# ittiam-systems/libxaac

Measured on AMD Instinct MI355X. Metric: decoded audio frames/s (1024-spl IMDCT + complex QMF + HQ SBR + parametric stereo, HE-AACv2), higher is better.
Workload: dtype int32

## Files before the change

### libxaac_amd/csrc/fx.h

```cpp
#ifndef XAAC_FX_H
#define XAAC_FX_H

#include <stdint.h>

#if defined(__HIPCC__)
#define FX_HD __host__ __device__ __forceinline__
#define FX_MEMBER __host__ __device__ __forceinline__
#else
#define FX_HD static inline
#define FX_MEMBER inline
#endif

#define FX_MAX32 ((int32_t)0x7fffffff)
#define FX_MIN32 ((int32_t)0x80000000)

FX_HD int32_t fx_add(int32_t a, int32_t b) { return (int32_t)((uint32_t)a + (uint32_t)b); }
FX_HD int32_t fx_sub(int32_t a, int32_t b) { return (int32_t)((uint32_t)a - (uint32_t)b); }
FX_HD int32_t fx_neg(int32_t a) { return (int32_t)(0u - (uint32_t)a); }
FX_HD int32_t fx_shlw(int32_t a, int n) { return (int32_t)((uint32_t)a << n); }

FX_HD int32_t fx_sat64(int64_t v) {
  if (v > (int64_t)FX_MAX32) return FX_MAX32;
  if (v < (int64_t)FX_MIN32) return FX_MIN32;
  return (int32_t)v;
}
FX_HD int32_t fx_add_sat(int32_t a, int32_t b) {
#if defined(__HIP_DEVICE_COMPILE__)
  return __builtin_elementwise_add_sat(a, b);
#else
  return fx_sat64((int64_t)a + (int64_t)b);
#endif
}
FX_HD int32_t fx_sub_sat(int32_t a, int32_t b) {
#if defined(__HIP_DEVICE_COMPILE__)
  return __builtin_elementwise_sub_sat(a, b);
#else
  return fx_sat64((int64_t)a - (int64_t)b);
#endif
}
FX_HD int32_t fx_neg_sat(int32_t a) {
#if defined(__HIP_DEVICE_COMPILE__)
  return __builtin_elementwise_sub_sat(0, a);
#else
  return a == FX_MIN32 ? FX_MAX32 : -a;
#endif
}
FX_HD int32_t fx_abs_sat(int32_t a) { return a == FX_MIN32 ? FX_MAX32 : (a < 0 ? -a : a); }
FX_HD int32_t fx_abs_nrm(int32_t a) { return a < 0 ? ~a : a; }

FX_HD int32_t fx_shl(int32_t a, int b) {
  b &= 0xff;
  return b > 31 ? 0 : fx_shlw(a, b);
}
FX_HD int32_t fx_shr(int32_t a, int b) {
  b &= 0xff;
  return a >> (b < 31 ? b : 31);
}
FX_HD int32_t fx_shl_sat(int32_t a, int b) {
  if (a > (FX_MAX32 >> b)) return FX_MAX32;
  if (a < (FX_MIN32 >> b)) return FX_MIN32;
  return fx_shlw(a, b);
}
FX_HD int32_t fx_shr_rnd(int32_t a, int b) {
  b &= 0xff;
  if (b >= 31) return a < 0 ? -1 : 0;
  if (b <= 0) return a;
  return fx_add_sat(a, (int32_t)1 << (b - 1)) >> b;
}
FX_HD int32_t fx_shl_dir_sat_limit(int32_t a, int b) {
  if (b < 0) {
    b = -b;
    if (b > 31) b = 31;
    return fx_shr(a, b);
  }
  return fx_shl_sat(a, b);
}
FX_HD int32_t fx_shl_dir(int32_t a, int b) { return b < 0 ? fx_shr(a, -b) : fx_shl(a, b); }
FX_HD int32_t fx_shr_dir(int32_t a, int b) { return b < 0 ? fx_shl(a, -b) : fx_shr(a, b); }

FX_HD int32_t fx_f2i_trunc(float v) { return (v >= 2147483648.0f || v < -2147483648.0f || v != v) ? FX_MIN32 : (int32_t)v; }

FX_HD int fx_norm32(int32_t a) {
  uint32_t u = (uint32_t)(a < 0 ? ~a : a);
  if (u == 0) return 31;
#if defined(__HIP_DEVICE_COMPILE__)
  return __clz((int)u) - 1;
#else
  return __builtin_clz(u) - 1;
#endif
}

FX_HD int16_t fx_round16(int32_t a) { return (int16_t)(fx_add_sat(a, 0x8000) >> 16); }
FX_HD int16_t fx_neg16(int16_t a) { return a == (int16_t)-32768 ? (int16_t)32767 : (int16_t)-a; }
FX_HD int16_t fx_sat16(int32_t a) { return a > 32767 ? (int16_t)32767 : (a < -32768 ? (int16_t)-32768 : (int16_t)a); }

FX_HD int32_t fx_mulhi(int32_t a, int32_t b) {
#if defined(__HIP_DEVICE_COMPILE__)
  return __mulhi(a, b);
#else
  return (int32_t)(((int64_t)a * (int64_t)b) >> 32);
#endif
}
FX_HD int32_t fx_mul32x16(int32_t a, int16_t b) { return fx_mulhi(a, (int32_t)((uint32_t)(uint16_t)b << 16)); }
FX_HD int32_t fx_mul32xhi(int32_t a, int32_t packed) { return fx_mulhi(a, (int32_t)((uint32_t)packed & 0xffff0000u)); }
FX_HD int32_t fx_mul32xlo(int32_t a, int32_t packed) { return fx_mulhi(a, (int32_t)((uint32_t)packed << 16)); }
FX_HD int32_t fx_mul32x16_nosh_sat(int32_t a, int16_t b) { return fx_sat64((int64_t)a * (int64_t)b); }
FX_HD int32_t fx_mul32(int32_t a, int32_t b) { return fx_mulhi(a, b); }
FX_HD int32_t fx_mul32_shl(int32_t a, int32_t b) { return fx_shlw(fx_mulhi(a, b), 1); }
FX_HD int32_t fx_mul32x16_shl(int32_t a, int16_t b) { return fx_shlw(fx_mul32x16(a, b), 1); }

#endif
```

### libxaac_amd/csrc/sbr_qmf.h

```cpp
#ifndef XAAC_SBR_QMF_H
#define XAAC_SBR_QMF_H

#include <stdint.h>
#include "fx.h"

#ifndef XQ_TABLES_DECLARED
#define XQ_TABLES_DECLARED
#if defined(__HIPCC__)
#define XAAC_TAB_QUAL static __device__ const
#include "tables_qmf.inc"
#undef XAAC_TAB_QUAL
#define XQ_T(name) xaac_qmf_##name
#else
#include "tables_qmf.inc"
#define XQ_T(name) xaac_qmf_##name
#endif
#endif

#ifndef XQ_ELD_TABLES_DECLARED
#define XQ_ELD_TABLES_DECLARED
#if defined(__HIPCC__)
#define XAAC_TAB_QUAL static __device__ const
#include "tables_qmf_eld.inc"
#undef XAAC_TAB_QUAL
#else
#include "tables_qmf_eld.inc"
#endif
#endif

#ifndef XQ_ESBR_TABLES_DECLARED
#define XQ_ESBR_TABLES_DECLARED
#if defined(__HIPCC__)
#define XAAC_TAB_QUAL static __device__ const
#include "tables_qmf_esbr.inc"
#undef XAAC_TAB_QUAL
#else
#include "tables_qmf_esbr.inc"
#endif
#endif

#if defined(__HIPCC__)
#define XQ_UNROLL _Pragma("unroll")
#else
#define XQ_UNROLL
#endif

FX_HD int32_t xq_mul(int32_t a, int16_t b) { return fx_mul32x16(a, b); }

struct XqW16 {
  typedef int16_t T;
  static FX_MEMBER int32_t madd(int32_t a, T wa, int32_t b, T wb) { return fx_add_sat(xq_mul(a, wa), xq_mul(b, wb)); }
  static FX_MEMBER int32_t msub(int32_t a, T wa, int32_t b, T wb) { return fx_sub_sat(xq_mul(a, wa), xq_mul(b, wb)); }
  static FX_MEMBER int32_t badd(int32_t a, T wa, int32_t b, T wb) { return fx_shlw(fx_add(xq_mul(a, wa), xq_mul(b, wb)), 1); }
  static FX_MEMBER int32_t bsub(int32_t a, T wa, int32_t b, T wb) { return fx_shlw(fx_sub(xq_mul(a, wa), xq_mul(b, wb)), 1); }
  static FX_MEMBER const T *w32() { return XQ_T(w_32); }
  static FX_MEMBER const T *w16() { return XQ_T(w_16); }
  template <int M> static FX_MEMBER const T *tw() { return M == 32 ? XQ_T(sin_cos_twiddle_l64) : XQ_T(sin_cos_twiddle_l32); }
  template <int M> static FX_MEMBER const T *alt() { return M == 32 ? XQ_T(alt_sin_twiddle_l64) : XQ_T(alt_sin_twiddle_l32); }
};
FX_HD int64_t xq_sub64_sat(int64_t a, int64_t b) {
  const int64_t d = (int64_t)((uint64_t)a - (uint64_t)b);
  if (((a ^ b) & INT64_MIN) != 0 && ((d ^ a) & INT64_MIN) != 0) return a < 0 ? INT64_MIN : INT64_MAX;
  return d;
}
FX_HD int64_t xq_add64(int64_t a, int64_t b) { return (int64_t)((uint64_t)a + (uint64_t)b); }
struct XqW32 {
  typedef int32_t T;
  static FX_MEMBER int32_t madd(int32_t a, T wa, int32_t b, T wb) { return (int32_t)(xq_add64((int64_t)a * wa, (int64_t)b * wb) >> 32); }
  static FX_MEMBER int32_t msub(int32_t a, T wa, int32_t b, T wb) { return (int32_t)(xq_sub64_sat((int64_t)a * wa, (int64_t)b * wb) >> 32); }
  static FX_MEMBER int32_t badd(int32_t a, T wa, int32_t b, T wb) { return fx_shlw((int32_t)(xq_add64((int64_t)a * wa, (int64_t)b * wb) >> 32), 1); }
  static FX_MEMBER int32_t bsub(int32_t a, T wa, int32_t b, T wb) {
    return fx_shlw((int32_t)((int64_t)((uint64_t)((int64_t)a * wa) - (uint64_t)((int64_t)b * wb)) >> 32), 1);
  }
  static FX_MEMBER const T *w32() { return XQ_T(esbr_w_32); }
  static FX_MEMBER const T *w16() { return XQ_T(esbr_w_16); }
  template <int M> static FX_MEMBER const T *tw() {
    return M == 32 ? XQ_T(esbr_sin_cos_twiddle_l64) : M == 16 ? XQ_T(esbr_sin_cos_twiddle_l32) : M == 12 ? XQ_T(esbr_sin_cos_twiddle_l24) : XQ_T(esbr_sin_cos_twiddle_l16);
  }
  template <int M> static FX_MEMBER const T *alt() {
    return M == 32 ? XQ_T(esbr_alt_sin_twiddle_l64) : M == 16 ? XQ_T(esbr_alt_sin_twiddle_l32) : M == 12 ? XQ_T(esbr_alt_sin_twiddle_l24) : XQ_T(esbr_alt_sin_twiddle_l16);
  }
};

template <class W = XqW16>
FX_HD void xq_radix4(const typename W::T *w, int32_t *x, int index1, int index) {
  const int h2 = 2 * index, l1 = 4 * index, l2 = 6 * index;
  XQ_UNROLL
  for (int b = 0; b < index1; b++) {
    XQ_UNROLL
    for (int i = 0; i < index; i++) {
      int32_t *p = x + 8 * index * b + 2 * i;
      const typename W::T si1 = w[6 * i], co1 = w[6 * i + 1], si2 = w[6 * i + 2], co2 = w[6 * i + 3], si3 = w[6 * i + 4],
                          co3 = w[6 * i + 5];
      int32_t xh0 = fx_add_sat(p[0], p[l1]), xl0 = fx_sub_sat(p[0], p[l1]);
      int32_t xh20 = fx_add_sat(p[h2], p[l2]), xl20 = fx_sub_sat(p[h2], p[l2]);
      int32_t xh1 = fx_add_sat(p[1], p[l1 + 1]), xl1 = fx_sub_sat(p[1], p[l1 + 1]);
      int32_t xh21 = fx_add_sat(p[h2 + 1], p[l2 + 1]), xl21 = fx_sub_sat(p[h2 + 1], p[l2 + 1]);
      int32_t xt0 = fx_sub_sat(xh0, xh20), yt0 = fx_sub_sat(xh1, xh21);
      int32_t xt1 = fx_add_sat(xl0, xl21), xt2 = fx_sub_sat(xl0, xl21);
      int32_t yt2 = fx_add_sat(xl1, xl20), yt1 = fx_sub_sat(xl1, xl20);
      p[0] = fx_add_sat(xh0, xh20);
      p[1] = fx_add_sat(xh1, xh21);
      p[l2] = W::badd(yt2, si3, xt2, co3);
      p[l2 + 1] = W::bsub(yt2, co3, xt2, si3);
      p[l1] = W::badd(yt0, si2, xt0, co2);
      p[l1 + 1] = W::bsub(yt0, co2, xt0, si2);
      p[h2] = W::badd(yt1, si1, xt1, co1);
      p[h2 + 1] = W::bsub(yt1, co1, xt1, si1);
    }
  }
}

FX_HD void xq_postradix4(int32_t *y, const int32_t *x) {
  XQ_UNROLL
  for (int k = 0; k < 2; k++) {
    const int h = XQ_T(dig_rev_table4_16)[k] >> 2;
    XQ_UNROLL
    for (int half = 0; half < 2; half++) {
      const int32_t *a = x + 16 * k + 8 * half;
      int32_t *o = y + h + 2 * half;
      int32_t xh0 = fx_add_sat(a[0], a[4]), xh1 = fx_add_sat(a[1], a[5]);
      int32_t xl0 = fx_sub_sat(a[0], a[4]), xl1 = fx_sub_sat(a[1], a[5]);
      int32_t yh0 = fx_add_sat(a[2], a[6]), yh1 = fx_add_sat(a[3], a[7]);
      int32_t yl0 = fx_sub_sat(a[2], a[6]), yl1 = fx_sub_sat(a[3], a[7]);
      o[0] = fx_add_sat(xh0, yh0);
      o[1] = fx_add_sat(xh1, yh1);
      o[8] = fx_add_sat(xl0, yl1);
      o[9] = fx_sub_sat(xl1, yl0);
      o[16] = fx_sub_sat(xh0, yh0);
      o[17] = fx_sub_sat(xh1, yh1);
      o[24] = fx_sub_sat(xl0, yl1);
      o[25] = fx_add_sat(xl1, yl0);
    }
  }
}

FX_HD void xq_postradix2(int32_t *y, const int32_t *x) {
  XQ_UNROLL
  for (int k = 0; k < 2; k++) {
    XQ_UNROLL
    for (int i = 0; i < 2; i++) {
// ... 551 lines not shown
```

### libxaac_amd/csrc/sbr_qmf_kernel.h

```cpp
#ifndef XAAC_SBR_QMF_KERNEL_H
#define XAAC_SBR_QMF_KERNEL_H

#include <hip/hip_runtime_api.h>
#include <stdint.h>

#include "../../include/xaac_amd.h"
#include "../../include/xaac_sbr.h"

#ifndef XAAC_QMF_WAVES
#define XAAC_QMF_WAVES 1
#endif
#define XAAC_QMF_BLOCK (64 * XAAC_QMF_WAVES)
#define XAAC_QMF_ANA_LDS_PER_WAVE (2 * 1312 * 2 + 32 + 64 * 65 * 4)
#define XAAC_QMF_SYN_LDS_PER_WAVE_LP 21376
#define XAAC_QMF_SYN_LDS_PER_WAVE_HQ (64 * 129 * 4)
#define XAAC_QMF_ANA_LDS (XAAC_QMF_WAVES * XAAC_QMF_ANA_LDS_PER_WAVE)
#define XAAC_QMF_SYN_LDS_LP (XAAC_QMF_WAVES * XAAC_QMF_SYN_LDS_PER_WAVE_LP)
#define XAAC_QMF_SYN_LDS_HQ (XAAC_QMF_WAVES * XAAC_QMF_SYN_LDS_PER_WAVE_HQ)

typedef struct XaacQmfAnaParams {
  int32_t n_ch, ch_fac, low_pow, usb, slot_stride;
  int32_t state_stride;
  int32_t qmf_ch_stride;
  const int16_t *pcm;
  xaac_qmf_ana_state *state;
  int32_t *qmf;
  const xaac_sbr_frame *frame;
  int32_t *zero_words;
  int32_t n_slots;
  const int16_t *refused;
} XaacQmfAnaParams;

typedef struct XaacQmfSynParams {
  int32_t n_ch, ch_fac, low_pow, lsb, usb, split, slot_stride;
  int32_t state_stride, qmf_ch_stride;
  int32_t scale_stride;
  int32_t per_ch_bands;
  int32_t down_sample;
  const int32_t *qmf;
  const int16_t *scale;
  xaac_qmf_syn_state *state;
  int16_t *pcm;
  int32_t pcm_ch_stride, pcm_sample_stride;
  int32_t *dbg;
  int32_t n_slots;
} XaacQmfSynParams;

#define XAAC_QMF_SYN_PAIR_BLOCK 128
#define XAAC_QMF_SYN_PAIR_LDS (2 * 42 * 65 * 4)
typedef struct XaacQmfSynPairParams {
  int32_t n;
  int32_t split;
  const int32_t *qmf[2];
  int32_t qmf_stride[2];
  const int16_t *scale[2];
  xaac_qmf_syn_state *state[2];
  int32_t state_stride[2];
  int16_t *pcm;
  int32_t *status;
  int32_t n_slots;
} XaacQmfSynPairParams;

#ifdef __cplusplus
extern "C" {
#endif
hipError_t xaac_launch_qmf_synthesis_pair(const XaacQmfSynPairParams *p, hipStream_t stream);
hipError_t xaac_launch_qmf_analysis(const XaacQmfAnaParams *p, int grid, hipStream_t stream);
#define XAAC_QMF_ELD_BLOCK 64
#define XAAC_QMF_ELD_LDS (4 * (288 + 512) * 2 + 64 * 65 * 4)
typedef struct XaacQmfEldChain {
  int32_t state_stride;
  int32_t pcm_ch_fac;
  const xaac_sbr_frame *frame;
  const int16_t *codec_usb;
  const int16_t *syn_par;
} XaacQmfEldChain;
hipError_t xaac_launch_qmf_analysis_eld(const xaac_qmf_ana_eld_batch *p, hipStream_t stream);
hipError_t xaac_launch_qmf_analysis_eld_chain(const xaac_qmf_ana_eld_batch *p, const XaacQmfEldChain *c, hipStream_t stream);
hipError_t xaac_launch_qmf_synthesis_eld_chain(const xaac_qmf_syn_eld_batch *p, const XaacQmfEldChain *c, hipStream_t stream);
#define XAAC_QMF_ELD_SYN_LDS (4 * 25 * 130 * 2)
hipError_t xaac_launch_qmf_synthesis_eld(const xaac_qmf_syn_eld_batch *p, hipStream_t stream);
hipError_t xaac_launch_qmf_synthesis(const XaacQmfSynParams *p, int grid, hipStream_t stream);
int xaac_qmf_blocks_per_cu(int which);
hipError_t xaac_warm_sbr_qmf(void);
#ifdef __cplusplus
}
#endif
#endif
```

### libxaac_amd/csrc/sbr_qmf_kernel.hip

```cpp
#include <hip/hip_runtime.h>
#include <stdint.h>

#include "sbr_qmf.h"
#include "sbr_qmf_kernel.h"

namespace {

constexpr int kHist = 288 + 1024;

__device__ __forceinline__ int ana_ring_pos(int wr, int a) {
  int p = wr + 32 + a;
  return p >= 320 ? p - 320 : p;
}

template <int NS = 32>
__device__ __forceinline__ int ana_phase_after_frame(int phase) {
  int f1 = phase, f2 = phase + 64;
  for (int s = 0; s < NS; s++) {
    f1 += 64;
    f2 += 64;
    int t = f1;
    f1 = f2;
    f2 = t;
    if (f2 > 640) {
// ... 438 lines not shown
      for (int c = 0; c < 2; c++) {
        if (2 * pair + c >= p.n_ch) break;
#pragma unroll
        for (int j = 0; j < HP; j++) {
          const int i = 2 * (lane + 64 * j);
          if (i < 9 * BLK) *reinterpret_cast<int32_t *>(&v[(c * VSLOTS + i / BLK) * VROW + i % BLK]) = hpair[c][j];
        }
      }
    }
    for (int c = 0; c < 2; c++) {
      const int ch = 2 * pair + c;
      if (ch >= p.n_ch) break;
      if (EARLY && hist_words) break;
      const xaac_qmf_syn_state *st = reinterpret_cast<const xaac_qmf_syn_state *>(
          reinterpret_cast<const char *>(p.state) + (size_t)ch * p.state_stride);
      const int d = __builtin_amdgcn_readfirstlane(d_v[c]);
      constexpr int HJ = 9 * BLK / 64;
      int16_t hist[HJ];
#pragma unroll
      for (int j = 0; j < HJ; j++) {
        const int i = lane + 64 * j;
        const int A = 9 - i / BLK;
        int pos = d + BLK * A + i % BLK;
        if (pos >= RING) pos -= RING;
        hist[j] = st->ring[pos];
      }
#pragma unroll
      for (int j = 0; j < HJ; j++) {
        const int i = lane + 64 * j;
        v[(c * VSLOTS + i / BLK) * VROW + i % BLK] = hist[j];
      }
    }
    asm volatile("s_waitcnt lgkmcnt(0)" ::: "memory");
    XQ_TIME(3);
    for (int c = 0; c < 2; c++) {
      const int ch = 2 * pair + c;
      if (ch >= p.n_ch) break;
      if (p.per_ch_bands && __builtin_amdgcn_readfirstlane(off_v[c])) continue;
      const int cf = p.pcm_sample_stride ? p.pcm_sample_stride : p.ch_fac;
      int16_t *dst = p.pcm_sample_stride ? p.pcm + (size_t)ch * p.pcm_ch_stride
                                         : p.pcm + (size_t)(ch / cf) * (NS * NC) * cf + (ch % cf);
      const int shift = LP ? 2 : 1;
      for (int s0 = 0; s0 < NS; s0 += 64 / NC) {
        const int s = DS ? s0 + (lane >> 5) : s0, k = DS ? (lane & 31) : lane;
        const int16_t *vs = v + (c * VSLOTS + 9 + s) * VROW + k;
        int32_t acc = 0x8000 >> shift;
#pragma unroll
        for (int A = 0; A < 10; A++) acc += (int32_t)vs[-VROW * A + NC * (A & 1)] * coef[A];
        dst[(size_t)(NC * s + k) * cf] = (int16_t)(fx_shl_sat(acc, shift) >> 16);
      }
    }
    XQ_TIME(4);
    for (int c = 0; c < 2; c++) {
      const int ch = 2 * pair + c;
      if (ch >= p.n_ch) break;
      if (p.per_ch_bands && __builtin_amdgcn_readfirstlane(off_v[c])) continue;
      xaac_qmf_syn_state *st =
          reinterpret_cast<xaac_qmf_syn_state *>(reinterpret_cast<char *>(p.state) + (size_t)ch * p.state_stride);
      const int d_new = (__builtin_amdgcn_readfirstlane(d_v[c]) + RING - (NS * BLK) % RING) % RING;
      const int ph_new = (st->phase + (64 * NS) % 640) % 640;
      for (int i = lane; i < RING; i += 64) {
        const int A = 1 + i / BLK;
        int pos = d_new + BLK * A + i % BLK;
        if (pos >= RING) pos -= RING;
        if (pos >= RING) pos -= RING;
        st->ring[pos] = v[(c * VSLOTS + 9 + NS - A) * VROW + i % BLK];
      }
      if (lane == 0) {
        st->drc_offset = (int16_t)d_new;
        st->phase = (int16_t)ph_new;
      }
    }
    XQ_TIME(5);
  }
#ifdef XS_PROFILE
  if (lane == 0 && p.dbg)
    for (int i = 0; i < 8; i++)
      atomicAdd(reinterpret_cast<unsigned long long *>(p.dbg) + 64 + (LP ? 0 : 8) + i, (unsigned long long)xq_acc[i]);
#endif
}

namespace {
__device__ __forceinline__ int32_t pair_rescale(int32_t v, int shl, int shr) { return (int32_t)((uint32_t)v << shl) >> shr; }
__device__ __forceinline__ int32_t clamp_med3(int32_t a, int32_t lo, int32_t hi) {
  int32_t r;
  asm("v_med3_i32 %0, %1, %2, %3" : "=v"(r) : "v"(a), "v"(lo), "v"(hi));
  return r;
}
typedef short xq_short2 __attribute__((ext_vector_type(2)));
}

#ifndef XQ_STAGGER_G
#define XQ_STAGGER_G 64
#define XQ_STAGGER_SLEEP 4
#endif
#ifndef XQ_STAGGER_FIRST
#define XQ_STAGGER_FIRST 1536
#endif
template <int NS = 32>
__global__ __launch_bounds__(XAAC_QMF_SYN_PAIR_BLOCK) void xaac_qmf_synthesis_pair_kernel(XaacQmfSynPairParams p) {
  constexpr int NH = NS / 2;
  extern __shared__ __attribute__((aligned(16))) char smem[];
  constexpr int RS = 65;
  constexpr int EROWS = 9 + 32 + 1;
  constexpr int RING = 1280;
  const int lane = threadIdx.x & 63;
  const int w = __builtin_amdgcn_readfirstlane(threadIdx.x >> 6);
  int32_t *tile_own = reinterpret_cast<int32_t *>(smem) + w * 32 * RS;
  const int32_t *tile_oth = reinterpret_cast<const int32_t *>(smem) + (1 - w) * 32 * RS;
  int32_t *E = reinterpret_cast<int32_t *>(smem);
  const int lch = lane >> 5, lrow = lane & 31;
  const int i = blockIdx.x;
  if (XQ_STAGGER_G > 1 && i < XQ_STAGGER_FIRST && (int)gridDim.x >= 3 * XQ_STAGGER_FIRST)
    for (int t = 0; t < i % XQ_STAGGER_G; t++) __builtin_amdgcn_s_sleep(XQ_STAGGER_SLEEP);
  typedef int xq_int4 __attribute__((ext_vector_type(4)));
  xaac_qmf_syn_state *st_w = reinterpret_cast<xaac_qmf_syn_state *>(reinterpret_cast<char *>(p.state[w]) + (size_t)i * p.state_stride[w]);
  const xaac_qmf_syn_state *st_o = reinterpret_cast<const xaac_qmf_syn_state *>(reinterpret_cast<const char *>(p.state[1 - w]) + (size_t)i * p.state_stride[1 - w]);
  const xq_int4 par0 = *reinterpret_cast<const xq_int4 *>(p.scale[0] + 8 * (size_t)i);
  const xq_int4 par1 = *reinterpret_cast<const xq_int4 *>(p.scale[1] + 8 * (size_t)i);
  const int d_old_v = st_w->drc_offset, d_oth_v = st_o->drc_offset;
  int32_t x[64];
  int32_t tmp[64];
#pragma unroll
  for (int r = 0; r < 64; r++) {
    const int c = r >> 5;
    tmp[r] = (r & 31) < NS ? (p.qmf[c] + (size_t)i * p.qmf_stride[c] + (size_t)(r & 31) * 128 + 64 * w)[lane] : 0;
  }
  const auto lo16 = [](int v) { return (int)(int16_t)v; };
  const auto hi16 = [](int v) { return v >> 16; };
  const int u0 = __builtin_amdgcn_readfirstlane(par0.x), u1 = __builtin_amdgcn_readfirstlane(par0.y);
  const int u2 = __builtin_amdgcn_readfirstlane(par0.z), u3 = __builtin_amdgcn_readfirstlane(par0.w);
  const int v0 = __builtin_amdgcn_readfirstlane(par1.x), v1 = __builtin_amdgcn_readfirstlane(par1.y);
  const int v2 = __builtin_amdgcn_readfirstlane(par1.z), v3 = __builtin_amdgcn_readfirstlane(par1.w);
  const int inactive0 = lo16(u3), inactive1 = lo16(v3);
  const int st_syn0 = hi16(u1), st_syn1 = hi16(v1);
  const int d_old = __builtin_amdgcn_readfirstlane(d_old_v);
  {
    const int d_oth = __builtin_amdgcn_readfirstlane(d_oth_v);
    if (((d_old | d_oth) & 127) != 0 || d_old < 0 || d_old >= RING || d_oth < 0 || d_oth >= RING) {
      if (threadIdx.x == 0 && p.status) p.status[i] = -1;
      return;
    }
  }
  {
    int shl[2][2], shr[2][2];
#pragma unroll
    for (int c = 0; c < 2; c++) {
      const int w0 = c ? v0 : u0, w1 = c ? v1 : u1, w2 = c ? v2 : u2;
      const int st_syn = hi16(w1), lsb = lo16(w2), usb = hi16(w2), hb = lo16(w1);
#pragma unroll
      for (int ov = 0; ov < 2; ov++) {
        const int lo_sf = ov ? hi16(w0) : lo16(w0);
        int sh = lane < lsb ? (st_syn - lo_sf) - 8 : (lane < usb ? (st_syn - hb) - 8 : 0);
        sh = sh > 31 ? 31 : (sh < -31 ? -31 : sh);
        shl[c][ov] = sh > 0 ? sh : 0;
        shr[c][ov] = sh < 0 ? -sh : 0;
      }
    }
#pragma unroll
    for (int c = 0; c < 2; c++) {
#pragma unroll
      for (int j = 0; j < 32; j++) {
        const bool ov = j < p.split;
        tile_own[RS * j + lane] = pair_rescale(tmp[32 * c + j], ov ? shl[c][1] : shl[c][0], ov ? shr[c][1] : shr[c][0]);
      }
      asm volatile("s_waitcnt lgkmcnt(0)" ::: "memory");
      if (lch == c) {
#pragma unroll
        for (int k = 0; k < 64; k++) x[k] = tile_own[RS * lrow + k];
      }
      asm volatile("s_waitcnt lgkmcnt(0)" ::: "memory");
    }
  }
  {
    int32_t t[64];
    if (w == 0)
      xq_cos_sin_mod_half<32, 0>(x, t);
    else
      xq_cos_sin_mod_half<32, 1>(x, t);
  }
  int16_t h_lo[9], h_hi[9];
#pragma unroll
  for (int A = 1; A <= 9; A++) {
    int pos = d_old + 128 * A;
    if (pos >= RING) pos -= RING;
    h_lo[A - 1] = st_w->ring[pos + lane];
    h_hi[A - 1] = st_w->ring[pos + 64 + lane];
  }
  int32_t o[64];
#pragma unroll
  for (int c = 0; c < 2; c++) {
    if (lch == c) {
#pragma unroll
      for (int k = 0; k < 64; k++) tile_own[RS * lrow + k] = x[k];
    }
    __syncthreads();
    if (lch == c) {
#pragma unroll
      for (int k = 0; k < 64; k++) o[k] = tile_oth[RS * lrow + k];
    }
    __syncthreads();
  }
  {
    const int ch = lane >> 5, slot = lane & 31;
    const int shift = -((ch ? st_syn1 : st_syn0) - 3) + 1;
    const int32_t hi = FX_MAX32 >> shift, lo = FX_MIN32 >> shift;
    int16_t *row = reinterpret_cast<int16_t *>(E + (ch * EROWS + 9 + slot) * RS);
    if (w == 0) {
#pragma unroll
      for (int c = 0; c < 64; c++) {
        int32_t a = fx_sub_sat(o[c], x[c]);
        a = clamp_med3(a, lo, hi);
        row[2 * c] = fx_round16(fx_shlw(a, shift));
      }
    } else {
#pragma unroll
      for (int c = 0; c < 64; c++) {
        int32_t a = fx_add_sat(x[63 - c], o[63 - c]);
        a = clamp_med3(a, lo, hi);
        row[2 * RS + 2 * c + 1] = fx_round16(fx_shlw(a, shift));
      }
    }
    if ((unsigned)(-(st_syn0 - 3) + 1) > 16u || (unsigned)(-(st_syn1 - 3) + 1) > 16u) {
      const int bx = shift & 31;
      if (w == 0) {
#pragma unroll
        for (int c = 0; c < 64; c++) row[2 * c] = fx_round16(fx_shl_sat(fx_sub_sat(o[c], x[c]), bx));
      } else {
#pragma unroll
        for (int c = 0; c < 64; c++) row[2 * RS + 2 * c + 1] = fx_round16(fx_shl_sat(fx_add_sat(x[63 - c], o[63 - c]), bx));
      }
    }
    int16_t *hrow = reinterpret_cast<int16_t *>(E + (w * EROWS) * RS);
#pragma unroll
    for (int A = 1; A <= 9; A++) {
      hrow[(9 - A) * 2 * RS + 2 * lane] = h_lo[A - 1];
      hrow[(10 - A) * 2 * RS + 2 * lane + 1] = h_hi[A - 1];
    }
  }
  __syncthreads();
  {
    xq_short2 cp[5];
#pragma unroll
    for (int j = 0; j < 5; j++) {
      cp[j].x = xaac_qmf_qmf_c[128 * j + lane];
      cp[j].y = xaac_qmf_qmf_c[128 * j + 64 + lane];
    }
    int32_t e[2][8 + NH];
#pragma unroll
    for (int c = 0; c < 2; c++)
#pragma unroll
      for (int q = 0; q < 8 + NH; q++) e[c][q] = E[(c * EROWS + 9 + NH * w - 8 + q) * RS + lane];
    int32_t *out = reinterpret_cast<int32_t *>(p.pcm) + (size_t)i * (64 * NS) + (64 * NH) * w + lane;
#pragma unroll
    for (int s = 0; s < NH; s++) {
      int32_t acc[2] = {0x4000, 0x4000};
#pragma unroll
      for (int c = 0; c < 2; c++)
#pragma unroll
        for (int j = 0; j < 5; j++) acc[c] = __builtin_amdgcn_sdot2(__builtin_bit_cast(xq_short2, e[c][8 + s - 2 * j]), cp[j], acc[c], false);
      const uint32_t l = (uint32_t)(uint16_t)(fx_add_sat(acc[0], acc[0]) >> 16), r = (uint32_t)(uint16_t)(fx_add_sat(acc[1], acc[1]) >> 16);
      if (!inactive0 && !inactive1) {
        out[64 * s] = (int32_t)(l | (r << 16));
      } else {
        int16_t *o16 = reinterpret_cast<int16_t *>(out + 64 * s);
        if (!inactive0) o16[0] = (int16_t)l;
        if (!inactive1) o16[1] = (int16_t)r;
      }
    }
  }
  if (w == 0 ? inactive0 : inactive1) return;
  {
    const int d_new = (d_old + RING - (NS * 128) % RING) % RING;
    const int ph_new = (st_w->phase + (64 * NS) % 640) % 640;
    const int16_t *hrow = reinterpret_cast<const int16_t *>(E + (w * EROWS) * RS);
    int16_t v_lo[10], v_hi[10];
#pragma unroll
    for (int A = 1; A <= 10; A++) {
      v_lo[A - 1] = hrow[(9 + NS - A) * 2 * RS + 2 * lane];
      v_hi[A - 1] = hrow[(10 + NS - A) * 2 * RS + 2 * lane + 1];
    }
#pragma unroll
    for (int A = 1; A <= 10; A++) {
      int pos = d_new + 128 * A;
      if (pos >= RING) pos -= RING;
      if (pos >= RING) pos -= RING;
      st_w->ring[pos + lane] = v_lo[A - 1];
      st_w->ring[pos + 64 + lane] = v_hi[A - 1];
    }
    if (lane == 0) {
      st_w->drc_offset = (int16_t)d_new;
      st_w->phase = (int16_t)ph_new;
    }
  }
}

extern "C" hipError_t xaac_launch_qmf_synthesis_pair(const XaacQmfSynPairParams *p, hipStream_t stream) {
  if (p->n_slots == 30)
    hipLaunchKernelGGL(xaac_qmf_synthesis_pair_kernel<30>, dim3(p->n), dim3(XAAC_QMF_SYN_PAIR_BLOCK), XAAC_QMF_SYN_PAIR_LDS, stream, *p);
  else
    hipLaunchKernelGGL(xaac_qmf_synthesis_pair_kernel<32>, dim3(p->n), dim3(XAAC_QMF_SYN_PAIR_BLOCK), XAAC_QMF_SYN_PAIR_LDS, stream, *p);
  return hipGetLastError();
}

namespace {
__device__ __forceinline__ int eld_phase(const xaac_qmf_ana_eld_state *st) {
  const int wr = st->wr;
  if (wr < 0 || wr > 288 || (wr & 31)) return -1;
  const int t = ((320 - wr) / 32) % 10;
  const int f1 = (t & 1) ? 32 * (t + 1) : 32 * t, f2 = (t & 1) ? 32 * t : 32 * t + 32;
  return (st->f1 == f1 && st->f2 == f2 && st->fp == 32 * (t & 1)) ? t : -1;
}
}

__global__ __launch_bounds__(XAAC_QMF_ELD_BLOCK) void xaac_qmf_analysis_eld_kernel(xaac_qmf_ana_eld_batch p, XaacQmfEldChain cn) {
  const auto state_of = [&](int ch) {
    return reinterpret_cast<xaac_qmf_ana_eld_state *>(reinterpret_cast<char *>(p.state) +
                                                      (size_t)ch * (cn.state_stride ? cn.state_stride : (int)sizeof(xaac_qmf_ana_eld_state)));
  };
  const int fac = cn.pcm_ch_fac > 1 ? cn.pcm_ch_fac : 1;
  extern __shared__ __attribute__((aligned(16))) char smem[];
  constexpr int H = 288 + 512;
  int16_t *hist = reinterpret_cast<int16_t *>(smem);
  int32_t *z = reinterpret_cast<int32_t *>(smem + 4 * H * 2);
  const int lane = threadIdx.x, ns = p.n_slots, quad = blockIdx.x;
  int32_t coef[5];
#pragma unroll
  for (int j = 0; j < 5; j++) coef[j] = xaac_qmf_eld_c3[lane + 64 * j];
  int phase[4];
  for (int c = 0; c < 4; c++) {
    const int ch = 4 * quad + c;
    int16_t *h = hist + c * H;
    phase[c] = -1;
    if (ch < p.n_ch) phase[c] = eld_phase(state_of(ch));
    if (phase[c] >= 0) {
      const xaac_qmf_ana_eld_state *st = state_of(ch);
      const int wr = st->wr;
      for (int a = lane; a < 288; a += 64) h[287 - a] = st->ring[ana_ring_pos(wr, a)];
      const int16_t *src = p.pcm + (size_t)(ch / fac) * 32 * ns * fac + ch % fac;
      for (int i = lane; i < 32 * ns; i += 64) h[288 + i] = src[(size_t)i * fac];
    } else {
      for (int i = lane; i < H; i += 64) h[i] = 0;
    }
    if (lane == 0 && p.status && ch < p.n_ch) p.status[ch] = phase[c] >= 0 ? 0 : -1;
  }
  __syncthreads();
  for (int r = 0; r < 64; r++) {
    const int s = r & 15;
    int32_t acc = 0;
    if (s < ns) {
      const int16_t *h = hist + (r >> 4) * H + 288 + 32 * s + 31 - lane;
#pragma unroll
      for (int j = 0; j < 5; j++) acc += (int32_t)h[-64 * j] * coef[j];
    }
    z[65 * r + lane] = acc;
  }
  __syncthreads();
  {
    int32_t in[64], sb[128], t[128];
#pragma unroll
    for (int k = 0; k < 64; k++) in[k] = z[65 * lane + k];
    int usb = p.usb;
    if (cn.frame) {
      const int chl = 4 * quad + (lane >> 4);
      if (chl < p.n_ch) {
        const xaac_sbr_frame *fr = cn.frame + chl;
        usb = fr->apply_processing ? fr->max_qmf_subband_aac
                                   : *reinterpret_cast<const int16_t *>(reinterpret_cast<const char *>(cn.codec_usb) + (size_t)chl * cn.state_stride);
        usb = usb < 0 ? 0 : (usb > 32 ? 32 : usb);
      }
    }
    xq_fwd_modulation(in, sb, t, usb, true);
#pragma unroll
    for (int k = 0; k < 32; k++) {
      z[65 * lane + k] = sb[k];
      z[65 * lane + 32 + k] = sb[64 + k];
    }
  }
  __syncthreads();
  for (int r = 0; r < 64; r++) {
// ... 199 lines not shown
```

### libxaac_amd/csrc/xaac_abi.cpp

```cpp
#include <hip/hip_runtime_api.h>
#include "build_id.h"

#include <cstdint>
#include <cstdlib>
#include <new>

#include "../../include/xaac_amd.h"
#include "imdct_kernel.h"
#include "sbr_qmf_kernel.h"
#include "sbr_core_kernel.h"
#include "sbr_ld_core_kernel.h"
#include "sbr_ps_kernel.h"
#include "limiter_kernel.h"
#include "esbr_qmf_kernel.h"
#include "usac_imdct_kernel.h"
#include "imdct960_kernel.h"
#include "imdct_ld_kernel.h"
#include "esbr_core_kernel.h"
#include "hbe_kernel.h"
#include "pvc_kernel.h"
#include "aac_tools_kernel.h"
#include "mc_sbr_kernel.h"
#include "out_map.h"
#include "out_map_kernel.h"
// ... 224 lines not shown
  const int w = hq ? 128 : 64;
  XaacQmfAnaParams pa = {};
  pa.n_ch = b->n_ch; pa.ch_fac = b->in_ch_fac; pa.low_pow = hq ? 0 : 1; pa.usb = 32; pa.slot_stride = w; pa.n_slots = ns;
  pa.state_stride = (int32_t)sizeof(xaac_sbr_state); pa.qmf_ch_stride = XAAC_SBR_X_ROWS * w; pa.pcm = b->pcm_in;
  pa.state = reinterpret_cast<xaac_qmf_ana_state *>(reinterpret_cast<char *>(b->state) + offsetof(xaac_sbr_state, ana_ring));
  pa.qmf = x + (2 + 6) * w; pa.zero_words = counters;
  if (hq) pa.frame = b->frame;
  if (ns == 30) {
    XaacSbrCoreParams sc = {};
    sc.n_ch = b->n_ch; sc.header = b->header; sc.frame = b->frame; sc.state = b->state; sc.syn_par = par; sc.qmf_slots = ns;
    const hipError_t e = xaac_launch_sbr_screen(&sc, c->stream);
    if (e != hipSuccess) return e;
    pa.refused = par;
  }
  return xaac_launch_qmf_analysis(&pa, qmf_grid(c, b->n_ch, hq ? 1 : 0), c->stream);
}

template <class B>
XaacSbrCoreParams sbr_core_params(const xaac_ctx *c, const B *b, int ns, int32_t *x, int16_t *par, int32_t *counters) {
  XaacSbrCoreParams pc = {};
  pc.n_ch = b->n_ch; pc.header = b->header; pc.frame = b->frame; pc.state = b->state; pc.x = x; pc.syn_par = par;
  pc.status = b->status; pc.qmf_slots = ns;
  pc.defer_count = counters; pc.work_counter = counters + 1; pc.num_cu = c->num_cu; pc.counters_zeroed = 1;
  return pc;
}

template <class B>
int32_t sbr_back(xaac_ctx *c, const B *b, bool hq, int ns, const int32_t *x, const int16_t *par) {
  const int w = hq ? 128 : 64;
  XaacQmfSynParams ps = {};
  ps.n_ch = b->n_ch; ps.ch_fac = b->out_ch_fac; ps.low_pow = hq ? 0 : 1; ps.split = 6; ps.n_slots = ns; ps.down_sample = b->down_sample ? 1 : 0;
  ps.slot_stride = w; ps.state_stride = (int32_t)sizeof(xaac_sbr_state); ps.qmf_ch_stride = XAAC_SBR_X_ROWS * w;
  ps.scale_stride = 8; ps.per_ch_bands = 1;
  ps.qmf = x + 2 * w; ps.scale = par; ps.pcm = b->pcm_out; ps.dbg = XAAC_DBG_BUF(b->status, b->n_ch);
  ps.state = reinterpret_cast<xaac_qmf_syn_state *>(reinterpret_cast<char *>(b->state) + offsetof(xaac_sbr_state, syn_ring));
  const int grid = qmf_grid(c, b->n_ch, hq ? 3 : 2);
  XAAC_TRY(xaac_launch_qmf_synthesis(&ps, grid, c->stream));
  return report(c, grid, XAAC_QMF_BLOCK, hq ? XAAC_QMF_SYN_LDS_HQ : XAAC_QMF_SYN_LDS_LP);
}

int32_t sbr_lp_run(xaac_ctx *c, const xaac_sbr_lp_batch *b, int ns) {
  if (!c || !b) return XAAC_FATAL_NULL_ARG;
  if (b->n_ch < 0) return XAAC_FATAL_BAD_ARG;
  if (ns == 30 && b->down_sample) return XAAC_FATAL_BAD_ARG;
  if (bad_ch_fac(b->in_ch_fac) || bad_ch_fac(b->out_ch_fac)) return XAAC_FATAL_BAD_ARG;
  if (b->n_ch % b->in_ch_fac || b->n_ch % b->out_ch_fac) return XAAC_FATAL_BAD_ARG;
  if (b->n_ch == 0) return XAAC_OK;
  if (!b->pcm_in || !b->header || !b->frame || !b->state || !b->pcm_out || !b->workspace) return XAAC_FATAL_NULL_ARG;
  if (b->workspace_bytes < xaac_sbr_lp_workspace_bytes(b->n_ch)) return XAAC_FATAL_BAD_ARG;
  XAAC_TRY(hipSetDevice(c->device));
  const SbrLpWs w(b->workspace, (size_t)b->n_ch);
  XAAC_TRY(sbr_front(c, b, false, ns, w.x, w.par, w.counters));
  const XaacSbrCoreParams pc = sbr_core_params(c, b, ns, w.x, w.par, w.counters);
  XAAC_TRY(xaac_launch_sbr_core_lp(&pc, c->stream));
  return sbr_back(c, b, false, ns, w.x, w.par);
}

int32_t sbr_hq_run(xaac_ctx *c, const xaac_sbr_hq_batch *b, int ns) {
  if (!c || !b) return XAAC_FATAL_NULL_ARG;
  if (b->n_ch < 0) return XAAC_FATAL_BAD_ARG;
  const bool with_ps = b->ps_frame != nullptr;
  if ((b->ps_frame == nullptr) != (b->ps_state == nullptr)) return XAAC_FATAL_BAD_ARG;
  if (ns == 30 && b->down_sample) return XAAC_FATAL_BAD_ARG;
  if (bad_ch_fac(b->in_ch_fac)) return XAAC_FATAL_BAD_ARG;
  if (!with_ps && bad_ch_fac(b->out_ch_fac)) return XAAC_FATAL_BAD_ARG;
  if (with_ps && b->down_sample) return XAAC_FATAL_BAD_ARG;
  if (b->n_ch % b->in_ch_fac || (!with_ps && b->n_ch % b->out_ch_fac)) return XAAC_FATAL_BAD_ARG;
  if (b->n_ch == 0) return XAAC_OK;
  if (!b->pcm_in || !b->header || !b->frame || !b->state || !b->pcm_out || !b->workspace) return XAAC_FATAL_NULL_ARG;
  if (b->workspace_bytes < xaac_sbr_hq_workspace_bytes(b->n_ch, with_ps)) return XAAC_FATAL_BAD_ARG;
  XAAC_TRY(hipSetDevice(c->device));
  const SbrHqWs w(b->workspace, (size_t)b->n_ch, with_ps);
  XAAC_TRY(sbr_front(c, b, true, ns, w.x, w.par_l, w.counters));
  XaacSbrCoreParams pc = sbr_core_params(c, b, ns, w.x, w.par_l, w.counters);
  pc.defer_list = w.defer_list;
  pc.narrow_only = b->max_band_hint == XAAC_SBR_NARROW_BANDS ? 1 : 0;
  XAAC_TRY(xaac_launch_sbr_core_hq(&pc, c->stream));
  if (!with_ps) return sbr_back(c, b, true, ns, w.x, w.par_l);
  XaacPsParams pp = {};
  pp.n_slots = ns; pp.n = b->n_ch; pp.x = w.x; pp.xr = w.xr; pp.header = b->header; pp.sbr_frame = b->frame; pp.frame = b->ps_frame;
  pp.state = b->ps_state; pp.sbr_state = b->state; pp.par_l = w.par_l; pp.par_r = w.par_r; pp.status = b->status; pp.dbg = XAAC_DBG_BUF(b->status, b->n_ch);
  XAAC_TRY(xaac_launch_ps(&pp, c->stream));
  XaacQmfSynPairParams pq = {};
  pq.n = b->n_ch; pq.split = 6; pq.n_slots = ns;
  pq.qmf[0] = w.x + 2 * 128; pq.qmf_stride[0] = 2 * XAAC_SBR_X_WORDS; pq.scale[0] = w.par_l;
  pq.state[0] = reinterpret_cast<xaac_qmf_syn_state *>(reinterpret_cast<char *>(b->state) + offsetof(xaac_sbr_state, syn_ring));
  pq.state_stride[0] = (int32_t)sizeof(xaac_sbr_state);
  pq.qmf[1] = w.xr; pq.qmf_stride[1] = 32 * 128; pq.scale[1] = w.par_r;
  pq.state[1] = reinterpret_cast<xaac_qmf_syn_state *>(reinterpret_cast<char *>(b->ps_state) + offsetof(xaac_ps_state, syn_ring_r));
  pq.state_stride[1] = (int32_t)sizeof(xaac_ps_state);
  pq.pcm = b->pcm_out; pq.status = b->status;
  XAAC_TRY(xaac_launch_qmf_synthesis_pair(&pq, c->stream));
  return report(c, b->n_ch, XAAC_QMF_SYN_PAIR_BLOCK, XAAC_QMF_SYN_PAIR_LDS);
}

int32_t limiter_run(xaac_ctx *c, const xaac_limiter_batch *b, const xaac_out_map *map) {
  if (!c || !b) return XAAC_FATAL_NULL_ARG;
  if (b->n_streams < 0 || b->frame_len < 1 || b->frame_len > 1024) return XAAC_FATAL_BAD_ARG;
  if (b->num_channels < 1 || b->num_channels > XAAC_LIM_MAX_CH) return XAAC_FATAL_BAD_ARG;
  if (b->stride < (int64_t)b->frame_len * b->num_channels) return XAAC_FATAL_BAD_ARG;
  if (b->n_streams == 0) return XAAC_OK;
  if (!b->samples || !b->qshift_adj || !b->state || !b->workspace) return XAAC_FATAL_NULL_ARG;
  if (b->workspace_bytes < xaac_peak_limiter_workspace_bytes(b->n_streams)) return XAAC_FATAL_BAD_ARG;
  XAAC_TRY(hipSetDevice(c->device));
  const LimiterWs w(b->workspace, (size_t)b->n_streams);
  XaacLimiterParams p = {};
  p.ws_gain = w.gain; p.ws_flag = w.flag;
  p.n_streams = b->n_streams; p.frame_len = b->frame_len; p.num_channels = b->num_channels; p.planar = b->planar ? 1 : 0;
  p.samples = b->samples; p.stride = b->stride; p.qshift_adj = b->qshift_adj; p.state = b->state; p.pcm16 = b->pcm16; p.status = b->status;
  p.dbg = reinterpret_cast<long long *>(XAAC_DBG_BUF(b->status, b->n_streams));
  if (map) {
    if (!b->pcm16) return XAAC_FATAL_NULL_ARG;
    p.map_kind = map->kind;
    if (map->kind == XAAC_OUT_MAP_NONE) return XAAC_FATAL_BAD_ARG;
    const int32_t rc = out_map_check(map, b->num_channels, b->pcm16, p.map_coef);
    if (rc != XAAC_OK) return rc;
  }
  XAAC_TRY(map ? xaac_launch_limiter_map(&p, c->stream) : xaac_launch_limiter(&p, c->stream));
  return report(c, b->n_streams, XAAC_LIM_BLOCK, XAAC_LIM_FRONT_LDS);
}

}

extern "C" {

const char *xaac_version(void) { return "libxaac_amd 0.4 gfx950 build " XAAC_BUILD_ID; }

int32_t xaac_create(xaac_ctx **out, int32_t device, void *hip_stream) {
  if (!out) return XAAC_FATAL_NULL_ARG;
  *out = nullptr;
  int n = 0;
  if (!hip_ok(hipGetDeviceCount(&n)) || n <= 0) return XAAC_FATAL_NO_DEVICE;
  if (device < 0 || device >= n) return XAAC_FATAL_BAD_ARG;
  if (!hip_ok(hipSetDevice(device))) return XAAC_FATAL_HIP;
  xaac_ctx *c = new (std::nothrow) xaac_ctx();
  if (!c) return XAAC_FATAL_HIP;
  c->device = device;
  c->owns_stream = false;
  c->stream = static_cast<hipStream_t>(hip_stream);
  if (!hip_stream) {
    if (!hip_ok(hipStreamCreateWithFlags(&c->stream, hipStreamNonBlocking))) {
      delete c;
      return XAAC_FATAL_HIP;
    }
    c->owns_stream = true;
  }
  hipDeviceProp_t prop;
  if (!hip_ok(hipGetDeviceProperties(&prop, device))) {
    if (c->owns_stream) (void)hipStreamDestroy(c->stream);
    delete c;
    return XAAC_FATAL_HIP;
  }
  c->num_cu = prop.multiProcessorCount > 0 ? prop.multiProcessorCount : 256;
  c->blocks_per_cu = xaac_imdct_blocks_per_cu();
  for (int i = 0; i < 4; i++) c->qmf_blocks_per_cu[i] = xaac_qmf_blocks_per_cu(i);
  c->last_grid = c->last_block = c->last_lds = 0;
  *out = c;
  return XAAC_OK;
}

int32_t xaac_destroy(xaac_ctx *c) {
  if (!c) return XAAC_FATAL_NULL_ARG;
  if (c->owns_stream) (void)hipStreamDestroy(c->stream);
  delete c;
  return XAAC_OK;
}

// ... 576 lines not shown
```

Before: 17.35 million.

## Micro-optimize QMF synthesis pair kernel: constant split, packed rounding, pipelined dot products

Several instruction-level tweaks go into the PS QMF synthesis pair kernel. The split index becomes a compile-time constant, and the twiddle multiply uses an opaque scalar-register hint. The clamp+shift+round sequence is replaced by a saturating round-with-shift plus packed 16-bit conversion. The output dot-product loop is software-pipelined, with packed stores done via a byte permute and separate paths for partially inactive channels. Together these aim to cut VALU instruction count and register pressure, at the cost of more inline asm and a hard requirement that split equals 6.

```diff
diff --git a/libxaac_amd/csrc/fx.h b/libxaac_amd/csrc/fx.h
--- a/libxaac_amd/csrc/fx.h
+++ b/libxaac_amd/csrc/fx.h
@@ -93,6 +93,8 @@
 FX_HD int16_t fx_round16(int32_t a) { return (int16_t)(fx_add_sat(a, 0x8000) >> 16); }
 FX_HD int16_t fx_neg16(int16_t a) { return a == (int16_t)-32768 ? (int16_t)32767 : (int16_t)-a; }
 FX_HD int16_t fx_sat16(int32_t a) { return a > 32767 ? (int16_t)32767 : (a < -32768 ? (int16_t)-32768 : (int16_t)a); }
+FX_HD int32_t fx_round16_shl_wide(int32_t a, int b) { return fx_add_sat(a, (int32_t)0x8000 >> b) >> (16 - b); }
+FX_HD int16_t fx_round16_shl_sat(int32_t a, int b) { return fx_sat16(fx_round16_shl_wide(a, b)); }
 
 FX_HD int32_t fx_mulhi(int32_t a, int32_t b) {
 #if defined(__HIP_DEVICE_COMPILE__)
diff --git a/libxaac_amd/csrc/sbr_qmf.h b/libxaac_amd/csrc/sbr_qmf.h
--- a/libxaac_amd/csrc/sbr_qmf.h
+++ b/libxaac_amd/csrc/sbr_qmf.h
@@ -57,6 +57,20 @@
   static FX_MEMBER const T *w16() { return XQ_T(w_16); }
   template <int M> static FX_MEMBER const T *tw() { return M == 32 ? XQ_T(sin_cos_twiddle_l64) : XQ_T(sin_cos_twiddle_l32); }
   template <int M> static FX_MEMBER const T *alt() { return M == 32 ? XQ_T(alt_sin_twiddle_l64) : XQ_T(alt_sin_twiddle_l32); }
+};
+FX_HD int32_t xq_opaque_word(int32_t c) {
+#if defined(__HIP_DEVICE_COMPILE__)
+  asm("" : "+s"(c));
+#endif
+  return c;
+}
+struct XqW16S : XqW16 {
+  static FX_MEMBER int32_t mul(int32_t a, T w) {
+    const int32_t c = (int32_t)((uint32_t)(uint16_t)w << 16);
+    return fx_mulhi(a, w < 0 ? xq_opaque_word(c) : c);
+  }
+  static FX_MEMBER int32_t badd(int32_t a, T wa, int32_t b, T wb) { return fx_shlw(fx_add(mul(a, wa), mul(b, wb)), 1); }
+  static FX_MEMBER int32_t bsub(int32_t a, T wa, int32_t b, T wb) { return fx_shlw(fx_sub(mul(a, wa), mul(b, wb)), 1); }
 };
 FX_HD int64_t xq_sub64_sat(int64_t a, int64_t b) {
   const int64_t d = (int64_t)((uint64_t)a - (uint64_t)b);
diff --git a/libxaac_amd/csrc/sbr_qmf_kernel.h b/libxaac_amd/csrc/sbr_qmf_kernel.h
--- a/libxaac_amd/csrc/sbr_qmf_kernel.h
+++ b/libxaac_amd/csrc/sbr_qmf_kernel.h
@@ -48,6 +48,7 @@
 
 #define XAAC_QMF_SYN_PAIR_BLOCK 128
 #define XAAC_QMF_SYN_PAIR_LDS (2 * 42 * 65 * 4)
+#define XAAC_QMF_SYN_PAIR_SPLIT 6
 typedef struct XaacQmfSynPairParams {
   int32_t n;
   int32_t split;
diff --git a/libxaac_amd/csrc/sbr_qmf_kernel.hip b/libxaac_amd/csrc/sbr_qmf_kernel.hip
--- a/libxaac_amd/csrc/sbr_qmf_kernel.hip
+++ b/libxaac_amd/csrc/sbr_qmf_kernel.hip
@@ -544,11 +544,6 @@
 
 namespace {
 __device__ __forceinline__ int32_t pair_rescale(int32_t v, int shl, int shr) { return (int32_t)((uint32_t)v << shl) >> shr; }
-__device__ __forceinline__ int32_t clamp_med3(int32_t a, int32_t lo, int32_t hi) {
-  int32_t r;
-  asm("v_med3_i32 %0, %1, %2, %3" : "=v"(r) : "v"(a), "v"(lo), "v"(hi));
-  return r;
-}
 typedef short xq_short2 __attribute__((ext_vector_type(2)));
 }
 
@@ -558,6 +553,11 @@
 #endif
 #ifndef XQ_STAGGER_FIRST
 #define XQ_STAGGER_FIRST 1536
+#endif
+#ifdef XQ_PHASE_MARKS
+#define XQ_MARK(i) asm volatile("; XQ_PHASE " #i)
+#else
+#define XQ_MARK(i)
 #endif
 template <int NS = 32>
 __global__ __launch_bounds__(XAAC_QMF_SYN_PAIR_BLOCK) void xaac_qmf_synthesis_pair_kernel(XaacQmfSynPairParams p) {
@@ -604,6 +604,7 @@
       return;
     }
   }
+  XQ_MARK(0);
   {
     int shl[2][2], shr[2][2];
 #pragma unroll
@@ -623,7 +624,7 @@
     for (int c = 0; c < 2; c++) {
 #pragma unroll
       for (int j = 0; j < 32; j++) {
-        const bool ov = j < p.split;
+        const bool ov = j < XAAC_QMF_SYN_PAIR_SPLIT;
         tile_own[RS * j + lane] = pair_rescale(tmp[32 * c + j], ov ? shl[c][1] : shl[c][0], ov ? shr[c][1] : shr[c][0]);
       }
       asm volatile("s_waitcnt lgkmcnt(0)" ::: "memory");
@@ -634,12 +635,13 @@
       asm volatile("s_waitcnt lgkmcnt(0)" ::: "memory");
     }
   }
+  XQ_MARK(1);
   {
     int32_t t[64];
     if (w == 0)
-      xq_cos_sin_mod_half<32, 0>(x, t);
+      xq_cos_sin_mod_half<32, 0, XqW16S>(x, t);
     else
-      xq_cos_sin_mod_half<32, 1>(x, t);
+      xq_cos_sin_mod_half<32, 1, XqW16S>(x, t);
   }
   int16_t h_lo[9], h_hi[9];
 #pragma unroll
@@ -650,6 +652,7 @@
     h_hi[A - 1] = st_w->ring[pos + 64 + lane];
   }
   int32_t o[64];
+  XQ_MARK(2);
 #pragma unroll
   for (int c = 0; c < 2; c++) {
     if (lch == c) {
@@ -663,24 +666,27 @@
     }
     __syncthreads();
   }
+  XQ_MARK(3);
   {
     const int ch = lane >> 5, slot = lane & 31;
     const int shift = -((ch ? st_syn1 : st_syn0) - 3) + 1;
-    const int32_t hi = FX_MAX32 >> shift, lo = FX_MIN32 >> shift;
     int16_t *row = reinterpret_cast<int16_t *>(E + (ch * EROWS + 9 + slot) * RS);
+    const int bq = (unsigned)shift <= 16u ? shift : 0;
     if (w == 0) {
 #pragma unroll
-      for (int c = 0; c < 64; c++) {
-        int32_t a = fx_sub_sat(o[c], x[c]);
-        a = clamp_med3(a, lo, hi);
-        row[2 * c] = fx_round16(fx_shlw(a, shift));
+      for (int c = 0; c < 64; c += 2) {
+        const xq_short2 v = __builtin_amdgcn_cvt_pk_i16(fx_round16_shl_wide(fx_sub_sat(o[c], x[c]), bq),
+                                                        fx_round16_shl_wide(fx_sub_sat(o[c + 1], x[c + 1]), bq));
+        row[2 * c] = v.x;
+        row[2 * c + 2] = v.y;
       }
     } else {
 #pragma unroll
-      for (int c = 0; c < 64; c++) {
-        int32_t a = fx_add_sat(x[63 - c], o[63 - c]);
-        a = clamp_med3(a, lo, hi);
-        row[2 * RS + 2 * c + 1] = fx_round16(fx_shlw(a, shift));
+      for (int c = 0; c < 64; c += 2) {
+        const xq_short2 v = __builtin_amdgcn_cvt_pk_i16(fx_round16_shl_wide(fx_add_sat(x[63 - c], o[63 - c]), bq),
+                                                        fx_round16_shl_wide(fx_add_sat(x[62 - c], o[62 - c]), bq));
+        row[2 * RS + 2 * c + 1] = v.x;
+        row[2 * RS + 2 * c + 3] = v.y;
       }
     }
     if ((unsigned)(-(st_syn0 - 3) + 1) > 16u || (unsigned)(-(st_syn1 - 3) + 1) > 16u) {
@@ -693,6 +699,7 @@
         for (int c = 0; c < 64; c++) row[2 * RS + 2 * c + 1] = fx_round16(fx_shl_sat(fx_add_sat(x[63 - c], o[63 - c]), bx));
       }
     }
+    XQ_MARK(4);
     int16_t *hrow = reinterpret_cast<int16_t *>(E + (w * EROWS) * RS);
 #pragma unroll
     for (int A = 1; A <= 9; A++) {
@@ -701,6 +708,7 @@
     }
   }
   __syncthreads();
+  XQ_MARK(5);
   {
     xq_short2 cp[5];
 #pragma unroll
@@ -714,23 +722,37 @@
 #pragma unroll
       for (int q = 0; q < 8 + NH; q++) e[c][q] = E[(c * EROWS + 9 + NH * w - 8 + q) * RS + lane];
     int32_t *out = reinterpret_cast<int32_t *>(p.pcm) + (size_t)i * (64 * NS) + (64 * NH) * w + lane;
-#pragma unroll
-    for (int s = 0; s < NH; s++) {
-      int32_t acc[2] = {0x4000, 0x4000};
-#pragma unroll
-      for (int c = 0; c < 2; c++)
-#pragma unroll
-        for (int j = 0; j < 5; j++) acc[c] = __builtin_amdgcn_sdot2(__builtin_bit_cast(xq_short2, e[c][8 + s - 2 * j]), cp[j], acc[c], false);
-      const uint32_t l = (uint32_t)(uint16_t)(fx_add_sat(acc[0], acc[0]) >> 16), r = (uint32_t)(uint16_t)(fx_add_sat(acc[1], acc[1]) >> 16);
-      if (!inactive0 && !inactive1) {
-        out[64 * s] = (int32_t)(l | (r << 16));
-      } else {
-        int16_t *o16 = reinterpret_cast<int16_t *>(out + 64 * s);
-        if (!inactive0) o16[0] = (int16_t)l;
-        if (!inactive1) o16[1] = (int16_t)r;
-      }
-    }
-  }
+    const auto slot_acc = [&](int c, int s) {
+      int32_t acc;
+      asm("v_dot2_i32_i16 %0, %1, %2, %3" : "=v"(acc) : "v"(e[c][8 + s]), "v"(__builtin_bit_cast(int32_t, cp[0])), "s"(0x4000));
+#pragma unroll
+      for (int j = 1; j < 5; j++) acc = __builtin_amdgcn_sdot2(__builtin_bit_cast(xq_short2, e[c][8 + s - 2 * j]), cp[j], acc, false);
+      return acc;
+    };
+    if (!inactive0 && !inactive1) {
+      int32_t a0 = slot_acc(0, 0), a1 = slot_acc(1, 0);
+#pragma unroll
+      for (int s = 0; s < NH; s++) {
+        int32_t n0 = 0, n1 = 0;
+        if (s + 1 < NH) n0 = slot_acc(0, s + 1), n1 = slot_acc(1, s + 1);
+        out[64 * s] = (int32_t)__builtin_amdgcn_perm((uint32_t)fx_add_sat(a1, a1), (uint32_t)fx_add_sat(a0, a0), 0x07060302u);
+        a0 = n0, a1 = n1;
+      }
+    } else if (!inactive0) {
+#pragma unroll
+      for (int s = 0; s < NH; s++) {
+        const int32_t a = slot_acc(0, s);
+        reinterpret_cast<int16_t *>(out + 64 * s)[0] = (int16_t)(fx_add_sat(a, a) >> 16);
+      }
+    } else if (!inactive1) {
+#pragma unroll
+      for (int s = 0; s < NH; s++) {
+        const int32_t a = slot_acc(1, s);
+        reinterpret_cast<int16_t *>(out + 64 * s)[1] = (int16_t)(fx_add_sat(a, a) >> 16);
+      }
+    }
+  }
+  XQ_MARK(6);
   if (w == 0 ? inactive0 : inactive1) return;
   {
     const int d_new = (d_old + RING - (NS * 128) % RING) % RING;
@@ -758,6 +780,7 @@
 }
 
 extern "C" hipError_t xaac_launch_qmf_synthesis_pair(const XaacQmfSynPairParams *p, hipStream_t stream) {
+  if (p->split != XAAC_QMF_SYN_PAIR_SPLIT) return hipErrorInvalidValue;
   if (p->n_slots == 30)
     hipLaunchKernelGGL(xaac_qmf_synthesis_pair_kernel<30>, dim3(p->n), dim3(XAAC_QMF_SYN_PAIR_BLOCK), XAAC_QMF_SYN_PAIR_LDS, stream, *p);
   else
diff --git a/libxaac_amd/csrc/xaac_abi.cpp b/libxaac_amd/csrc/xaac_abi.cpp
--- a/libxaac_amd/csrc/xaac_abi.cpp
+++ b/libxaac_amd/csrc/xaac_abi.cpp
@@ -330,7 +330,7 @@
   pp.state = b->ps_state; pp.sbr_state = b->state; pp.par_l = w.par_l; pp.par_r = w.par_r; pp.status = b->status; pp.dbg = XAAC_DBG_BUF(b->status, b->n_ch);
   XAAC_TRY(xaac_launch_ps(&pp, c->stream));
   XaacQmfSynPairParams pq = {};
-  pq.n = b->n_ch; pq.split = 6; pq.n_slots = ns;
+  pq.n = b->n_ch; pq.split = XAAC_QMF_SYN_PAIR_SPLIT; pq.n_slots = ns;
   pq.qmf[0] = w.x + 2 * 128; pq.qmf_stride[0] = 2 * XAAC_SBR_X_WORDS; pq.scale[0] = w.par_l;
   pq.state[0] = reinterpret_cast<xaac_qmf_syn_state *>(reinterpret_cast<char *>(b->state) + offsetof(xaac_sbr_state, syn_ring));
   pq.state_stride[0] = (int32_t)sizeof(xaac_sbr_state);
```

Result: no change. 17.35 million (median of 2 runs) (-0.0%).
